# songlab-cal/CherryML

Hardware: AMD Instinct MI355X
Metric: cherry-pairs/sec (whole node) per EM iter (higher is better)
Workload: dtype f64

## Files before the change

cherryml_amd/bank.py:

```python
from typing import Optional, Tuple

import numpy as np

from . import _lib
from ._lib import CB_NO_SYNC, CB_NORMALIZE, CB_PTR_DEVICE, CB_TRAIN_RESUME


def _as_f64(a, shape=None) -> np.ndarray:
    a = np.ascontiguousarray(a, dtype=np.float64)
    if shape is not None and tuple(a.shape) != tuple(shape):
        raise ValueError(f"expected shape {tuple(shape)}, got {a.shape}")
    return a


class CherryBank:

    def __init__(self, t, C, device: int = 0, dtype: str = "f64", per_bucket_products: bool = False):
        self._h = None
        codes = {"f64": _lib.CB_F64, "f32": _lib.CB_F32, "mixed": _lib.CB_MIXED}
        if dtype not in codes:
            raise ValueError(f'dtype must be "f64", "f32" or "mixed", got {dtype!r}')
        self.dtype = dtype
        code = codes[dtype]
        cflags = _lib.CB_PER_BUCKET_PRODUCTS if per_bucket_products else 0
# ... 109 lines not shown
        _lib.check(_lib.load().cb_last_timings(self._h, ms.ctypes.data, ms.size), "cb_last_timings")
        return dict(zip(self.TIMING_NAMES, ms.tolist()))

    def timing_means(self) -> dict:
        import ctypes as Ct
        ms = np.zeros(len(self.TIMING_NAMES))
        calls = Ct.c_int(0)
        _lib.check(_lib.load().cb_timing_sums(self._h, ms.ctypes.data, ms.size, Ct.byref(calls)),
                   "cb_timing_sums")
        k = max(calls.value, 1)
        out = dict(zip(self.TIMING_NAMES, (ms / k).tolist()))
        out["calls"] = calls.value
        return out

    def last_sweeps(self) -> int:
        return int(_lib.load().cb_last_sweeps(self._h))

    def eigh_counters(self) -> dict:
        v = np.zeros(4, dtype=np.int32)
        _lib.check(_lib.load().cb_eigh_counters(self._h, v.ctypes.data, 4), "cb_eigh_counters")
        return {"planned_solves": int(v[0]), "stalls": int(v[1]), "last_sweeps": int(v[2]), "record_spins": int(v[3])}

    def epoch_times(self, num_epochs: int) -> np.ndarray:
        s = np.zeros(int(num_epochs))
        _lib.check(_lib.load().cb_train_epoch_times(self._h, s.ctypes.data, s.size), "cb_train_epoch_times")
        return s

    def last_kernel_form(self) -> int:
        return int(_lib.load().cb_last_kernel_form(self._h))

    def last_bank_form(self) -> dict:
        v = int(_lib.load().cb_last_bank_form(self._h))
        return {"fused": bool(v & 1), "waves_per_tile": 8 if v & 2 else 4, "bucket_sum_first": bool(v & 4),
                "time_basis": bool(v & 8)}

    def time_basis_info(self) -> dict:
        import ctypes as Ct
        n = np.zeros(5, dtype=np.int32)
        rho = Ct.c_double(0.0)
        _lib.check(_lib.load().cb_time_basis_info(self._h, n.ctypes.data, Ct.byref(rho)), "cb_time_basis_info")
        return {"forward_skeleton": int(n[0]), "direct": int(n[1]), "gradient_skeleton": int(n[2]), "builds": int(n[3]),
                "repeated_epochs": int(n[4]), "rho_max": float(rho.value)}

    def _shape_Q(self, Q, pi):
        Q = _as_f64(Q).reshape(self.L, self.S, self.S)
        pi = _as_f64(pi).reshape(self.L, self.S)
        return Q, pi

    def loss_grad(self, Q, pi, normalize: bool = True, want_grad: bool = True
                  ) -> Tuple[np.ndarray, Optional[np.ndarray]]:
        Q, pi = self._shape_Q(Q, pi)
        loss = np.zeros(self.L)
        dQ = np.zeros_like(Q) if want_grad else None
        rc = _lib.load().cb_loss_grad(self._h, Q.ctypes.data, pi.ctypes.data,
                                      CB_NORMALIZE if normalize else 0, loss.ctypes.data,
                                      dQ.ctypes.data if want_grad else None)
        _lib.check(rc, "cb_loss_grad")
        return loss, dQ

    def expm_bank(self, Q, pi=None) -> np.ndarray:
        Q = _as_f64(Q).reshape(self.L, self.S, self.S)
        pi_ptr = None
        if pi is not None:
            pi = _as_f64(pi).reshape(self.L, self.S)
            pi_ptr = pi.ctypes.data
        P = np.zeros((self.L, self.B, self.S, self.S))
        _lib.check(_lib.load().cb_expm_bank(self._h, Q.ctypes.data, pi_ptr, 0, P.ctypes.data),
# ... 84 lines not shown
```

cherryml_amd/csrc/cb_internal.hip.h:

```cpp
#pragma once
#include "../../include/cherrybank.h"

#include <hip/hip_runtime.h>

#include <algorithm>
#include <atomic>
#include <chrono>
#include <cmath>
#include <cstdarg>
#include <cstdio>
#include <cstdlib>
#include <cstring>
#include <string>
#include <vector>

int cb_fail(int code, const char *fmt, ...);
#define fail cb_fail

#define HIP_TRY(expr)                                                                   \
  do {                                                                                  \
    hipError_t e_ = (expr);                                                             \
    if (e_ != hipSuccess)                                                               \
      return fail(e_ == hipErrorOutOfMemory ? CB_ENOMEM : CB_EHIP, "%s failed: %s (%s:%d)", \
                  #expr, hipGetErrorString(e_), __FILE__, __LINE__);                    \
// ... 5 lines not shown
struct CbSpectral {
  int S = 0, LD = 0;
  const double *A = nullptr, *U = nullptr, *lam = nullptr, *dsq = nullptr, *sigma = nullptr;
};
int cb_internal_spectral(cb_handle h, CbSpectral *out);

int cb_launch_bank_fused(int variant, int kg, const void *args, int grid, hipStream_t stream, hipEvent_t stop);

#define CB_TB_RS_MAX 24
#define CB_TB_RG_MAX 40
struct CbTimeBasisHost {
  int B = 0, ns = 0, nd = 0, ng = 0;
  double rho_max = 0.0;
  double res_s = 0.0, res_g = 0.0;
  std::vector<int> kind;
  std::vector<int> skel_s, direct, skel_g;
  std::vector<double> tf, tg;
  std::vector<double> Ls, Lg;
};
bool cb_tb_build(int B, const double *t, double rho_max, CbTimeBasisHost &out);
struct CbTbEwArgs {
  int S, LD, B, ns, nd, ng;
  int nsmall;
  const double *Ct;
  const double *Psi;
  const double *A;
  const double *t;
  const double *Ls, *Lg;
  double *Gh;
  float *Gh32;
  double *loss_part;
  double inv_n;
  const unsigned long long *skip;
};
int cb_tb_launch_tables(int LD, int ns, int nd, int ng, const double *tf, const double *tg, const double *lam, double *F, double *E,
                        double *H, const unsigned long long *skip, hipStream_t stream);
#define CB_TB_LDS_MAX (144u << 10)
size_t cb_tb_ew_lds_bytes(int B, int ns, int ng);
bool cb_tb_supported(int B, int LD, int ns, int ng);
int cb_tb_prepare_ew(int B, int ns, int ng, size_t *cache);
int cb_tb_launch_ew(const CbTbEwArgs &a, hipStream_t stream, hipEvent_t stop, int *nparts);

static inline const char *cb_test_hook(const char *name) {
  const char *on = getenv("CB_TEST_HOOKS");
  return (on && on[0] == '1') ? getenv(name) : nullptr;
}

struct CbDevBufs {
  std::vector<void *> ptrs;
  ~CbDevBufs() {
    for (void *p : ptrs)
      if (p) (void)hipFree(p);
  }
  template <typename T>
  T *up(const T *host, size_t count, int &rc) {
    void *q = nullptr;
    if (rc != CB_OK) return nullptr;
    if (hipMalloc(&q, (count ? count : 1) * sizeof(T)) != hipSuccess) {
      rc = fail(CB_ENOMEM, "device allocation failed");
      return nullptr;
    }
    ptrs.push_back(q);
    if (host && count && hipMemcpyAsync(q, host, count * sizeof(T), hipMemcpyHostToDevice, 0) != hipSuccess)
      rc = fail(CB_EHIP, "upload failed");
    return static_cast<T *>(q);
  }
};
```

cherryml_amd/csrc/cherrybank.hip:

```cpp
#include "cb_internal.hip.h"

#include "common.hip.h"
#include "jacobi_block.hip.h"
#include "jacobi_wave.hip.h"
#include "large_bank.hip.h"
#include "small_bank.hip.h"
#include "train_small.hip.h"
#include "train_large.hip.h"
#include "general_small.hip.h"
#include "general_large.hip.h"
#include "eigh_planned.hip.h"

#define CB_ABI_VERSION 2

static thread_local std::string g_err;

int cb_fail(int code, const char *fmt, ...) {
  char buf[512];
  va_list ap;
  va_start(ap, fmt);
  vsnprintf(buf, sizeof buf, fmt, ap);
  va_end(ap);
  g_err = buf;
  return code;
// ... 181 lines not shown
      h->tb_next_pending = false;
      int rc = tb_install(h, B, std::move(nb), -1.0);
      if (rc != CB_OK || h->tb_failed) return rc;
      took = true;
    }
    if ((stale && !took) || !tb_in_range(h, B, two_sigma)) return tb_rebuild(h, B, two_sigma);
    return CB_OK;
  }
  double warn = 1.6;
  int lead = CB_TB_LEAD;
  if (const char *w = cb_test_hook("CB_TB_TEST_WARN")) sscanf(w, "%lf %d", &warn, &lead);
  if (h->tb_next_pending && epoch >= h->tb_next_epoch) {
    CbTimeBasisHost nb = h->tb_next.get();
    h->tb_next_pending = false;
    int rc = tb_install(h, B, std::move(nb), -1.0);
    if (rc != CB_OK || h->tb_failed) return rc;
  }
  if (!h->tb_next_pending && !tb_in_range(h, B, two_sigma, warn)) {
    std::vector<double> t(h->t_live_host.begin(), h->t_live_host.begin() + B);
    const double rho = two_sigma * tb_growth();
    h->tb_next = std::async(std::launch::async, [t, rho, B]() {
      CbTimeBasisHost nb;
      if (!cb_tb_build(B, t.data(), rho, nb)) nb = CbTimeBasisHost{};
      return nb;
    });
    h->tb_next_pending = true;
    h->tb_next_epoch = epoch + lead;
  }
  return CB_OK;
}

struct LargeBankForm {
  bool tb = false;
  bool fused = false;
  bool accum = false;
  int kg = 1;
  int n_parts = 1;
  int tiles_k3 = 0;
  int test_no_claim = 0;
  double phi_delta = 0;
};

static LargeBankForm choose_large_form(const cb_bank *h, int B, bool Pd, bool want_grad, bool planned_now) {
  static const int streams = getenv("CB_BANK_STREAMS") ? std::min(4, std::max(1, atoi(getenv("CB_BANK_STREAMS")))) : 1;
  const char *tb_hook = cb_test_hook("CB_BANK_TB"), *fused_hook = cb_test_hook("CB_BANK_FUSED"),
             *unfused_hook = cb_test_hook("CB_BANK_UNFUSED"), *k3_hook = cb_test_hook("CB_BANK_K3"),
             *kg_hook = cb_test_hook("CB_BANK_KG"), *no_claim_hook = cb_test_hook("CB_BANK_TEST_NO_CLAIM"),
             *phi_z_hook = cb_test_hook("CB_PHI_Z");
  const int LD = h->LD, tm = (LD + LG_TM - 1) / LG_TM, tn = (LD + LG_TN - 1) / LG_TN;
  const bool f32 = h->dtype == CB_F32 && !Pd;
  LargeBankForm f;
  const bool form_hooks = fused_hook || unfused_hook || k3_hook || kg_hook || no_claim_hook;
  f.tb = h->sym_counts && !h->per_bucket_products && !h->tb_block && !h->tb_failed && !Pd && want_grad && h->tb_Ls[0] &&
         streams == 1 && (h->dtype == CB_F64 || h->dtype == CB_MIXED) &&
         (tb_hook ? atoi(tb_hook) != 0 : (!form_hooks && B >= CB_TB_MIN_B));
  if (f.tb && planned_now && h->tb.B != B) f.tb = false;
  {
    const size_t nb16 = (size_t)LD / 16, cap = (size_t)B * tm * tn;
    if (nb16 * (nb16 + 1) > cap) f.tb = false;
  }
  f.fused = !Pd && want_grad && !unfused_hook && streams == 1 && h->bank_queue && (fused_hook || B >= CB_BANK_FUSED_MIN_B);
  f.accum = h->sym_counts && !h->per_bucket_products && !Pd && want_grad && h->Yk && streams == 1 && h->dtype == CB_F64 &&
            (k3_hook ? atoi(k3_hook) == 0 : (B >= CB_BANK_SUM_FIRST_MIN_B && h->phi_delta >= 4e-3));
  f.tiles_k3 = f.accum ? 0 : h->sym_counts ? tn * (tn + 1) / 2 : tm * tn;
  f.phi_delta = h->phi_delta;
  if (phi_z_hook) f.phi_delta *= atof(phi_z_hook) / 0.1;
  f.kg = (B < CB_BANK_KG2_MAX_B && !f32) ? 2 : 1;
  if (kg_hook) f.kg = atoi(kg_hook) == 1 ? 1 : 2;
  if (Pd) f.kg = 1;
  if (streams > 1 && h->dtype == CB_F64 && !Pd && want_grad && B >= 4 * streams && !h->comm && !h->profile) f.n_parts = streams;
  f.test_no_claim = no_claim_hook ? 1 : 0;
  return f;
}

struct LargeCall {
  int B;
  const double *t;
  double inv_n;
  double *loss, *dQ, *Pd;
  bool dA_padded, planned_now;
  const unsigned long long *skipw;
  size_t LL;
  int tiles, tiles_k1;
};

template <typename T1, typename TG>
struct BankBufs {
  const T1 *Ut, *A, *F, *Ct;
  TG *Gt, *T;
  const TG *U;
  int variant;
};
template <typename T1, typename TG>
// ... 39 lines not shown
  const int LD = h->LD;
  const LossArgs la{h->loss_part, nparts, h->S, h->dsq, h->dirsum, c.inv_n, c.loss, c.skipw};
  const dim3 red_grid((unsigned)((c.LL + 255) / 256) + 1);
  if (f.accum) {
    hipLaunchKernelGGL(ky_reduce_loss<TG>, red_grid, dim3(256), 0, h->stream, src, YArgs{LD, c.B, c.t, h->E, h->Yk}, la);
    K4Args gl{h->S, LD, h->Yk, h->U, h->Lk, nullptr, nullptr, nullptr};
    gl.skip = c.skipw;
    gl.ystride = c.LL;
    launch_sg(h, gl, 0, 0.0, 0.0, nullptr, nullptr, 1 + CB_PHI_TERMS);
    LAUNCH_STOP(k3_stop, kphi_combine<CB_PHI_TERMS>, dim3((unsigned)((c.LL + 255) / 256)), dim3(256), 0, h->stream, LD, h->Lk,
                h->lam, f.phi_delta, h->Mt, c.skipw);
  } else {
    hipLaunchKernelGGL(k3_reduce_loss<TG>, red_grid, dim3(256), 0, h->stream, src, nb, c.LL, h->Mt, sym_ld, la);
  }
  enqueue_k4(h, c, c.skipw, stop_event(h, EV_K4));
  HIP_TRY(hipGetLastError());
  return CB_OK;
}

template <typename TG>
static int enqueue_tb_bank(cb_bank *h, const LargeBankForm &f, const LargeCall &c) {
  constexpr bool mixed = std::is_same_v<TG, float>;
  const CbTimeBasisHost &bas = h->tb;
  const int S = h->S, LD = h->LD, set = h->tb_set, nf = bas.ns + bas.nd, ng = bas.ng;
  const auto bb = bank_bufs<double, TG>(h);
  if (!c.planned_now && cb_tb_launch_tables(LD, bas.ns, bas.nd, ng, h->tb_tf[set], h->tb_tg[set], h->lam, h->F, h->E, h->H,
                                            c.skipw, h->stream) != 0)
    return fail(CB_EHIP, "tb_tables: launch failed");
  double *psi_buf = mixed ? reinterpret_cast<double *>(h->T32) : h->T;
  K1Args<double> k1{S, LD, nf, h->Vc, h->A, h->tb_tf[set], h->F, h->sigma, h->Ct, psi_buf, h->loss_part, c.inv_n, h->dsq, nullptr, c.skipw};
  LAUNCH_STOP(stop_event(h, EV_K1), (k1_pt_loss_gt<double, double, false, 1, true>), dim3(c.tiles_k1 * nf), dim3(LG4_THREADS), 0,
              h->stream, k1);
  const CbTbEwArgs ew{S, LD, c.B, bas.ns, bas.nd, ng, c.B - bas.nd, h->Ct, psi_buf, h->A, c.t, h->tb_Ls[set], h->tb_Lg[set], h->Gt,
                      mixed ? h->Gt32 : nullptr, h->loss_part, c.inv_n, c.skipw};
  int ew_parts = 0;
  if (cb_tb_launch_ew(ew, h->stream, stop_event(h, EV_K2), &ew_parts) != 0) return fail(CB_EHIP, "tb_ew: launch failed");
  if (mixed) launch_cast_f32(h, c, 0);
  const K2Args<TG> k2{LD, bb.Gt, bb.U, bb.T, c.skipw};
  const K3Args<TG> k3{LD, ng, bb.T, bb.U, h->tb_tg[set], h->lam, h->E, h->H, bb.Gt, 1, c.skipw};
  hipLaunchKernelGGL((k2_t_eq_g_u<TG, 1>), dim3(c.tiles * ng), dim3(LG4_THREADS), 0, h->stream, k2);
  LAUNCH_STOP(stop_event(h, EV_K3), (k3_w_phi<TG, 1>), dim3(c.tiles_k1 * ng), dim3(LG4_THREADS), 0, h->stream, k3);
  return enqueue_tail<TG>(h, f, c, bb.Gt, ng, ew_parts, LD, nullptr);
}

template <typename T1, typename TG>
static int enqueue_fused_bank(cb_bank *h, const LargeBankForm &f, const LargeCall &c) {
  const int S = h->S, LD = h->LD, B = c.B;
  const auto bb = bank_bufs<T1, TG>(h);
  const int total = B * (c.tiles_k1 + c.tiles + f.tiles_k3), grid = std::min(h->bank_slots / f.kg, total);
  const int sym = h->sym_counts ? 1 : 0;
  if (h->profile && h->profile_now) h->ev_rec[EV_K1] = h->ev_rec[EV_K2] = false;
  const hipEvent_t bank_stop = stop_event(h, EV_K3);
  static_assert(sizeof(K123Args<float, float>) == sizeof(K123Args<double, double>) &&
                sizeof(K123Args<double, float>) == sizeof(K123Args<double, double>), "one argument block for all");
  const K123Args<T1, TG> a{{S, LD, B, bb.Ut, bb.A, c.t, bb.F, h->sigma, bb.Ct, bb.Gt, h->loss_part, c.inv_n, h->dsq, nullptr, c.skipw},
                           {LD, bb.Gt, bb.U, bb.T, c.skipw},
                           {LD, B, bb.T, bb.U, c.t, h->lam, h->E, h->H, bb.Gt, sym, c.skipw},
                           {h->bank_queue, B, c.tiles_k1, c.tiles, f.tiles_k3, h->bank_claims, f.test_no_claim}};
  auto *dst = reinterpret_cast<K123Args<T1, TG> *>(h->bank_args);
  hipLaunchKernelGGL((lg_tables<K123Args<T1, TG>>), dim3((unsigned)(((size_t)B * LD + 255) / 256)), dim3(256), 0, h->stream, LD, B,
                     c.t, h->lam, h->sigma, h->F, h->E, h->H, a, dst, grid);
  if (std::is_same_v<TG, float>) launch_cast_f32(h, c, (size_t)B * LD);
  if (cb_launch_bank_fused(bb.variant, f.kg, dst, grid, h->stream, bank_stop) != 0) return fail(CB_EHIP, "k123_bank: launch failed");
  return enqueue_tail<TG>(h, f, c, f.accum ? bb.T : bb.Gt, B, B * c.tiles_k1, h->sym_counts ? LD : 0, nullptr);
}

template <typename T1, typename TG>
static int enqueue_split_bank(cb_bank *h, const LargeBankForm &f, const LargeCall &c) {
  const int S = h->S, LD = h->LD, B = c.B;
  const auto bb = bank_bufs<T1, TG>(h);
  launch_tables(h, c);
  if (std::is_same_v<TG, float>) launch_cast_f32(h, c, (size_t)B * LD);
  const K1Args<T1, TG> k1{S, LD, B, bb.Ut, bb.A, c.t, bb.F, h->sigma, bb.Ct, bb.Gt, h->loss_part, c.inv_n, h->dsq, c.Pd, c.skipw};
// ... 62 lines not shown
  HIP_TRY(hipGetLastError());
  return CB_OK;
}

static int large_eval(cb_bank *h, bool normalize, double *lossd, double *out, bool dA_padded, double *Pd,
                      bool reuse_eigh = false, const EighPlan *plan = nullptr, int plan_first_slot = 0) {
  const int LD = h->LD, B = Pd ? h->B : h->Bl;
  const bool planned_now = plan && h->have_prev;
  LargeBankForm f = choose_large_form(h, B, Pd != nullptr, out != nullptr, planned_now);
  const unsigned long long *skipw = planned_now ? h->ectl + (f.tb ? EC_SKIP : EC_STALL) : nullptr;
  int rc = CB_OK;
  if (planned_now) {
    TbTableArgs tbt;
    if (f.tb) tbt = TbTableArgs{h->tb.ns, h->tb.nd, h->tb.ng, h->tb_tf[h->tb_set], h->tb_tg[h->tb_set], h->F, h->E, h->H};
    rc = enqueue_planned_solve(h, *plan, ++h->eseq, plan_first_slot, f.tb ? h->tb.rho_max : 0.0, tbt);
  }
  else if (!(reuse_eigh && h->have_prev)) rc = large_eigh(h, true);
  if (rc != CB_OK) return rc;
  if (f.tb && !planned_now) {
    double sg = 0.0;
    HIP_TRY(hipMemcpyAsync(&sg, h->sigma, sizeof sg, hipMemcpyDeviceToHost, h->stream));
    HIP_TRY(hipStreamSynchronize(h->stream));
    if (!tb_in_range(h, B, 2.0 * sg)) {
      rc = tb_rebuild(h, B, 2.0 * sg);
      if (rc != CB_OK) return rc;
      if (h->tb_failed) f.tb = false;
    }
  }
  if (f.tb) {
    f.fused = f.accum = false;
    f.kg = 1;
  }
  h->bank_tb = f.tb;
  h->bank_fused = f.fused;
  h->bank_accum = f.accum;
  h->bank_kg = f.kg;
  SlowScope scope_bank("large_eval: tables, bank, K4 enqueue");
  if (!planned_now) mark(h, EV_EIGH);
  const int tm = (LD + LG_TM - 1) / LG_TM, tn = (LD + LG_TN - 1) / LG_TN;
  const LargeCall c{B, Pd ? h->t : h->t_live, normalize ? 1.0 / (h->comm ? h->n_global[0] : h->n_host[0]) : 1.0, lossd, out, Pd,
                    dA_padded, planned_now, skipw, (size_t)LD * LD, tm * tn, tn * (tn + 1) / 2};
  if (f.tb) return h->dtype == CB_MIXED ? enqueue_tb_bank<float>(h, f, c) : enqueue_tb_bank<double>(h, f, c);
  if (f.n_parts > 1) return enqueue_stream_split_bank(h, f, c);
  return with_format(h, Pd != nullptr, [&](auto t1, auto tg) {
    using T1 = decltype(t1);
    using TG = decltype(tg);
    return f.fused ? enqueue_fused_bank<T1, TG>(h, f, c) : enqueue_split_bank<T1, TG>(h, f, c);
  });
}

static int large_loss_grad(cb_bank *h, const double *Qd, const double *pid, bool normalize,
                           double *lossd, double *dQd, double *Pd, bool reuse_eigh = false) {
  const size_t LL = (size_t)h->LD * h->LD;
  if (!(reuse_eigh && h->have_prev))
    hipLaunchKernelGGL(lg_build_A, dim3((unsigned)((LL + 255) / 256)), dim3(256), 0, h->stream, h->S, h->LD,
                       Qd, pid, h->A, h->dsq);
  return large_eval(h, normalize, lossd, dQd, false, Pd, reuse_eigh);
}

static int general_run(cb_bank *h, const double *Qd, int flags, double *lossd, double *dQd,
                       double *Pd);
static int finish_call(cb_bank *h, int flags) {
  if ((flags & CB_PTR_DEVICE) && (flags & CB_NO_SYNC)) return CB_OK;
  HIP_TRY(hipStreamSynchronize(h->stream));
  return CB_OK;
}
// ... 221 lines not shown
  h->profile_every = enable > 1 ? enable : 1;
  h->profile_now = h->profile;
  for (double &x : h->t_sum) x = 0.0;
  h->t_calls = 0;
  h->t_pending = false;
  h->t_pending2 = false;
  return CB_OK;
}

extern "C" int cb_timing_sums(cb_handle h, double *ms_sum, int n, int *calls) {
  if (!h || !ms_sum || !calls) return fail(CB_EINVAL, "cb_timing_sums: NULL argument");
  fold_pending(h);
  for (int i = 0; i < n; ++i) ms_sum[i] = i < CB_T_COUNT ? h->t_sum[i] : 0.0;
  *calls = h->t_calls;
  return CB_OK;
}

extern "C" int cb_last_sweeps(cb_handle h) { return h ? h->last_sweeps : 0; }
#ifdef CB_CLOCK_STAMP
extern "C" int cb_debug_clock_stamps(unsigned long long *out) {
  return hipMemcpyFromSymbol(out, HIP_SYMBOL(cb_clock_stamps), sizeof(unsigned long long) * 3 * 4096 * 6) == hipSuccess ? 0 : -1;
}
#endif

extern "C" int cb_eigh_counters(cb_handle h, int *counts, int n) {
  if (!h || !counts || n < 0) return fail(CB_EINVAL, "cb_eigh_counters: NULL argument");
  const int v[4] = {h->planned_solves, h->planned_stalls, h->last_sweeps,
                    (int)std::min<long long>(h->record_spins, 0x7fffffff)};
  for (int i = 0; i < n && i < 4; ++i) counts[i] = v[i];
  return CB_OK;
}
extern "C" int cb_last_kernel_form(cb_handle h) { return h ? h->last_form : 0; }
extern "C" int cb_last_bank_form(cb_handle h) {
  return h ? (h->bank_fused ? 1 : 0) | (h->bank_kg == 2 ? 2 : 0) | (h->bank_accum ? 4 : 0) | (h->bank_tb ? 8 : 0) : 0;
}
extern "C" int cb_time_basis_info(cb_handle h, int *n, double *rho_max) {
  if (!h || !n || !rho_max) return fail(CB_EINVAL, "cb_time_basis_info: NULL argument");
  n[0] = h->tb.ns;
  n[1] = h->tb.nd;
  n[2] = h->tb.ng;
  n[3] = h->tb_builds;
  n[4] = h->tb_stale_epochs;
  *rho_max = h->tb.rho_max;
  return CB_OK;
}

extern "C" int cb_last_timings(cb_handle h, double *ms, int n) {
  if (!h || !ms) return fail(CB_EINVAL, "cb_last_timings: NULL argument");
  for (int i = 0; i < n; ++i) ms[i] = 0.0;
  double v[CB_T_COUNT];
  int rc = read_phase_times(h, v);
  if (rc != CB_OK) return rc;
  for (int i = 0; i < n && i < CB_T_COUNT; ++i) ms[i] = v[i];
  return CB_OK;
}

static int read_phase_times(cb_bank *h, double (&v)[CB_T_COUNT]) {
  for (double &x : v) x = 0.0;
  if (!h->ev_rec[EV_START]) return fail(CB_EINVAL, "cb_last_timings: no profiled call recorded");
  {
    int last = EV_START;
    for (int i = 0; i <= CB_T_COUNT; ++i)
      if (h->ev_rec[i] && i != EV_END && i != EV_AR) last = i;
    if (h->ev_rec[EV_AR]) last = EV_AR;
    HIP_TRY(hipEventSynchronize(h->ev[last]));
  }
  auto span = [&](int a, int b) -> double {
// ... 24 lines not shown
```

cherryml_amd/csrc/handle_host.hip.h:

```cpp
#pragma once
#include <hip/hip_ext.h>
#include <future>
struct EighSlot {
  int cap = 12;
  int nsq = 0;
  int band_after = 0;
  int so = 0;
  int expect_run = 1, expect_order = 12, expect_sq = 2;
};
struct EighPlan {
  int lead_band = 1;
  int nslots = 0;
  EighSlot slot[EC_MAXREC];
};
struct cb_bank {
  int dev = 0, S = 0, L = 0, B = 0;
  int B_cap = 0;
  hipStream_t xstream[3] = {};
  hipEvent_t ev_fork = nullptr, ev_join[3] = {};
  int tr_epochs = 0;
  uint64_t tr_sig = 0;
  int last_form = 0;
  double tr_pow_b1 = 1.0, tr_pow_b2 = 1.0;
  int dtype = CB_F64;
// ... 36 lines not shown
  unsigned long long poll_seq = 0;
  unsigned long long *ectl = nullptr, *epin = nullptr;
  double *epart = nullptr;
  bool begin_folded = false;
  double *sigma_home = nullptr;
  double *sigma2 = nullptr;
  unsigned long long eseq = 0;
  bool planned_unavailable = false;
  int planned_solves = 0, planned_stalls = 0;
  long long record_spins = 0;
  std::vector<double> epoch_seconds;
  EighPlan eplan;
  int k3_chunk = 0, k3_nchunks = 0;
  double *Yk = nullptr, *Lk = nullptr;
  double phi_delta = 0.0;
  unsigned int *bank_queue = nullptr;
  unsigned char *bank_args = nullptr;
  int bank_slots = 0;
  int bank_claims = 0;
  bool bank_fused = false;
  int bank_kg = 1;
  bool bank_accum = false;
  CbTimeBasisHost tb;
  int tb_set = 0;
  double *tb_Ls[2] = {}, *tb_Lg[2] = {}, *tb_tf[2] = {}, *tb_tg[2] = {};
  std::future<CbTimeBasisHost> tb_next;
  bool tb_next_pending = false;
  int tb_next_epoch = 0;
  size_t tb_ew_lds[4] = {0, 0, 0, 0};
  int tb_builds = 0, tb_stale_epochs = 0;
  bool tb_failed = false;
  bool tb_block = false;
  bool bank_tb = false;
  int last_sweeps = 0;
  double *gn_scratch = nullptr, *gn_partial = nullptr;
  int gn_nw = 0;
  struct {
    double *Qn = nullptr, *QT = nullptr, *colsum = nullptr, *alpha = nullptr, *R = nullptr, *RT = nullptr, *E = nullptr,
           *ET = nullptr, *G = nullptr, *GT = nullptr, *Xbar = nullptr, *lpart = nullptr;
    int *nsq = nullptr;
    int cap_slots = 0;
  } gl;
  std::vector<double> t_host, t_live_host;
  bool have_prev = false;
  double *ws_ptr[16] = {};
  size_t ws_cap[16] = {};
  char *pin = nullptr;
  size_t pin_cap = 0, pin_off = 0;
  bool profile = false;
  int profile_every = 1;
  bool profile_now = false;
  hipEvent_t ev[CB_T_COUNT + 1] = {};
  bool ev_rec[CB_T_COUNT + 1] = {};
  double t_sum[CB_T_COUNT] = {};
  int t_calls = 0;
  bool t_pending = false;
  hipEvent_t ev2[CB_T_COUNT + 1] = {};
  bool ev_rec2[CB_T_COUNT + 1] = {};
  bool t_pending2 = false;
};

static void swap_event_sets(cb_bank *h) {
  for (int i = 0; i <= CB_T_COUNT; ++i) {
    std::swap(h->ev[i], h->ev2[i]);
    std::swap(h->ev_rec[i], h->ev_rec2[i]);
  }
// ... 97 lines not shown
```

cherryml_amd/csrc/large_bank.hip.h:

```cpp
#pragma once
#include "common.hip.h"
#include <type_traits>

#define LG_TM 80
#define LG_TN 80
#define LG_KT 16
#define LG4_THREADS 256

typedef float f4 __attribute__((ext_vector_type(4)));
template <typename T> struct Mfma;
template <> struct Mfma<double> {
  typedef d4 acc_t;
  typedef double2 vec_t;
  static constexpr int VEC = 2;
  static __device__ __forceinline__ acc_t mma(double a, double b, acc_t c) { return mfma_f64(a, b, c); }
  static __device__ __forceinline__ int row(int hi, int r) { return hi + 4 * r; }
  static constexpr int RSTEP = 4;
};
template <> struct Mfma<float> {
  typedef f4 acc_t;
  typedef float4 vec_t;
  static constexpr int VEC = 4;
  static __device__ __forceinline__ acc_t mma(float a, float b, acc_t c) {
    return __builtin_amdgcn_mfma_f32_16x16x4f32(a, b, c, 0, 0, 0);
// ... 28 lines not shown
__device__ __forceinline__ PanelSrc<T> lg4_panel_src(const T *P, int ld, int cols_total, int c0, int tid) {
  constexpr int VEC = Panel<T>::VEC, NL = Panel<T>::NL;
  const int kr = tid >> 4, cq = tid & 15;
  PanelSrc<T> s;
  s.rsrc = __builtin_amdgcn_make_buffer_rsrc(const_cast<T *>(P), 0, 0x7fffffff, 0x00027000);
#pragma unroll
  for (int u = 0; u < NL; ++u) s.voff[u] = (kr * ld + min(c0 + VEC * (cq + 16 * u), cols_total - VEC)) * (int)sizeof(T);
  return s;
}
template <typename T, bool SCALE>
__device__ __forceinline__ void lg4_load_panel(const PanelSrc<T> &src, int ld, int k0, typename Mfma<T>::vec_t (&reg)[Panel<T>::NL],
                                               const T *__restrict__ kscale, T &sc, int tid) {
  typedef typename Mfma<T>::vec_t vec_t;
  constexpr int NL = Panel<T>::NL;
  const int soff = k0 * ld * (int)sizeof(T);
#pragma unroll
  for (int u = 0; u < NL; ++u)
    reg[u] = __builtin_bit_cast(vec_t, __builtin_amdgcn_raw_buffer_load_b128(src.rsrc, src.voff[u], soff, 0));
  if (SCALE) sc = kscale[k0 + (tid >> 4)];
}
template <typename T, bool SCALE>
__device__ __forceinline__ void lg4_store_panel(T *s, const typename Mfma<T>::vec_t (&reg)[Panel<T>::NL], T sc, int tid) {
  typedef typename Mfma<T>::vec_t vec_t;
  constexpr int VEC = Panel<T>::VEC, NL = Panel<T>::NL, LAST = Panel<T>::LAST;
  const int kr = tid >> 4, cq = tid & 15;
  T *row = s + kr * LG_TM + VEC * cq;
#pragma unroll
  for (int u = 0; u < NL; ++u) {
    vec_t v = reg[u];
    if (SCALE) vec_scale(v, sc);
    if (u < NL - 1 || cq < LAST) *reinterpret_cast<vec_t *>(row + 16 * VEC * u) = v;
  }
}
struct BankHooks {
  unsigned int *deferred = nullptr;
  unsigned int *draw = nullptr;
  int *drawn_lds = nullptr;
};

template <int KG> __device__ __forceinline__ bool lg_owns_acc(int kg, int j) { return KG == 1 || (kg == 0) == (j < 3); }
template <int KG> __device__ __forceinline__ bool lg_owns_ax0(int kg) { return KG == 1 || kg == 1; }
template <int KG> __device__ __forceinline__ bool lg_owns_ax1(int kg) { return KG == 1 || kg == 0; }

template <typename T, bool SCALE, bool ZERO = true, int KG = 1>
__device__ __forceinline__ void lg4_gemm_tile(const GemmOperands<T> &g, int m0, int n0, T *sA, T *sB,
                                              typename Mfma<T>::acc_t (&acc)[5], typename Mfma<T>::acc_t &ax0,
                                              typename Mfma<T>::acc_t &ax1, int tid = threadIdx.x,
                                              const BankHooks &hooks = BankHooks{}) {
  static_assert(KG == 1 || KG == 2, "one or two K-groups of four waves");
  static_assert(KG == 1 || ZERO, "the accumulate-onto form exists for four waves only");
  typedef typename Mfma<T>::acc_t acc_t;
  typedef typename Mfma<T>::vec_t vec_t;
  const int wv = __builtin_amdgcn_readfirstlane(tid >> 6);
  const int kg = KG == 1 ? 0 : wv >> 2, wave = wv & 3, t4 = tid & 255;
  const int lane = tid & 63, lo = lane & 15, hi = lane >> 4;
  T *const sAll = sA;
  if (KG > 1) {
    sA += kg * (4 * LG_KT * LG_TM);
    sB += kg * (4 * LG_KT * LG_TM);
  }
  if (ZERO) {
#pragma unroll
    for (int j = 0; j < 5; ++j) acc[j] = acc_t{};
    ax0 = acc_t{};
    ax1 = acc_t{};
  }
  vec_t ra[Panel<T>::NL], rb[Panel<T>::NL];
  T sc = T(1), one = T(1);
  const int nk = g.K / LG_KT, nit = (nk + KG - 1) / KG;
  const PanelSrc<T> srcA = lg4_panel_src<T>(g.A, g.lda, g.M, m0, t4), srcB = lg4_panel_src<T>(g.B, g.ldb, g.N, n0, t4);
  if (kg < nk) {
    lg4_load_panel<T, SCALE>(srcA, g.lda, kg * LG_KT, ra, g.kscale, sc, t4);
    lg4_load_panel<T, false>(srcB, g.ldb, kg * LG_KT, rb, nullptr, one, t4);
  }
  __syncthreads();
  if (kg < nk) {
    lg4_store_panel<T, SCALE>(sA, ra, sc, t4);
    lg4_store_panel<T, false>(sB, rb, one, t4);
  }
  unsigned int *deferred = hooks.deferred;
  if (deferred) __builtin_amdgcn_s_waitcnt(0x0F70);
  __syncthreads();
  if (deferred && tid == 0) __hip_atomic_fetch_add(deferred, 1u, __ATOMIC_RELAXED, __HIP_MEMORY_SCOPE_AGENT);
  int drawn = -1;
  const int draw_it = nit > 2 ? 2 / KG : 0;
  for (int it = 0; it < nit; ++it) {
    const int kt = it * KG + kg;
    const T *cA = sA + (it & 1) * (LG_KT * LG_TM), *cB = sB + (it & 1) * (LG_KT * LG_TN);
    if (hooks.draw && it == draw_it && tid == 0)
      drawn = (int)__hip_atomic_fetch_add(hooks.draw, 1u, __ATOMIC_RELAXED, __HIP_MEMORY_SCOPE_AGENT);
    const bool more = kt + KG < nk;
    if (more) {
      lg4_load_panel<T, SCALE>(srcA, g.lda, (kt + KG) * LG_KT, ra, g.kscale, sc, t4);
      lg4_load_panel<T, false>(srcB, g.ldb, (kt + KG) * LG_KT, rb, nullptr, one, t4);
    }
    if (KG == 1 || kt < nk) {
#pragma unroll
      for (int s = 0; s < LG_KT / 4; ++s) {
        const T av = cA[(4 * s + hi) * LG_TM + 16 * wave + lo];
        const T a4 = cA[(4 * s + hi) * LG_TM + 64 + lo];
        T bv[5];
#pragma unroll
        for (int j = 0; j < 5; ++j) bv[j] = cB[(4 * s + hi) * LG_TN + 16 * j + lo];
#pragma unroll
        for (int j = 0; j < 5; ++j) acc[j] = Mfma<T>::mma(av, bv[j], acc[j]);
        const T bx = cB[(4 * s + hi) * LG_TN + 16 * wave + lo];
        ax0 = Mfma<T>::mma(a4, bx, ax0);
        if ((it & 3) == wave) ax1 = Mfma<T>::mma(a4, bv[4], ax1);
      }
    }
    if (more) {
      lg4_store_panel<T, SCALE>(sA + ((it + 1) & 1) * (LG_KT * LG_TM), ra, sc, t4);
      lg4_store_panel<T, false>(sB + ((it + 1) & 1) * (LG_KT * LG_TN), rb, one, t4);
    }
    __syncthreads();
  }
  if (KG == 1) {
    if (wave != 0) {
#pragma unroll
      for (int r = 0; r < 4; ++r) sA[(wave - 1) * 256 + r * 64 + lane] = ax1[r];
    }
    __syncthreads();
    if (wave == 0) {
#pragma unroll
      for (int r = 0; r < 4; ++r) ax1[r] += (sA[r * 64 + lane] + sA[256 + r * 64 + lane]) + sA[512 + r * 64 + lane];
    } else {
      ax1 = acc_t{};
    }
  } else {
    T *px = sAll, *to1 = sAll + 7 * 256, *to0 = to1 + 12 * 256;
    if (wv != 0) {
#pragma unroll
      for (int r = 0; r < 4; ++r) px[(wv - 1) * 256 + r * 64 + lane] = ax1[r];
    }
    if (kg == 0) {
#pragma unroll
      for (int r = 0; r < 4; ++r) {
        to1[(wave * 3 + 0) * 256 + r * 64 + lane] = acc[3][r];
        to1[(wave * 3 + 1) * 256 + r * 64 + lane] = acc[4][r];
        to1[(wave * 3 + 2) * 256 + r * 64 + lane] = ax0[r];
      }
    } else {
#pragma unroll
      for (int r = 0; r < 4; ++r) {
        to0[(wave * 3 + 0) * 256 + r * 64 + lane] = acc[0][r];
        to0[(wave * 3 + 1) * 256 + r * 64 + lane] = acc[1][r];
        to0[(wave * 3 + 2) * 256 + r * 64 + lane] = acc[2][r];
      }
// ... 229 lines not shown
  if (EXPM || RAW) return;
  __syncthreads();
  lossacc = wave_sum(lossacc);
  double *sRed = reinterpret_cast<double *>(sAB);
  if (lane == 0) sRed[wv] = lossacc;
  __syncthreads();
  if (tid == 0) {
    double l = (sRed[0] + sRed[1]) + (sRed[2] + sRed[3]);
    if (KG == 2) l += (sRed[4] + sRed[5]) + (sRed[6] + sRed[7]);
    a.loss_part[vid] = l;
  }
  CB_STAMP_FINISH(0);
}

template <typename T, typename TG = T, bool EXPM = false, int KG = 1, bool RAW = false>
__global__ __launch_bounds__(LG4_THREADS * KG, 4) void k1_pt_loss_gt(K1Args<T, TG> a) {
  if (a.skip && *a.skip != 0ull) return;
  __shared__ T sAB[KG * 4 * LG_KT * LG_TM];
  const int tilesN = (a.LD + LG_TN - 1) / LG_TN, tiles = tilesN * (tilesN + 1) / 2;
  const int vid = xcd_swizzle(blockIdx.x, gridDim.x);
  const int b = vid / tiles;
  k1_tile<T, TG, EXPM, false, KG, RAW>(a, b, vid - b * tiles, sAB, threadIdx.x);
}

template <typename T>
struct K2Args {
  int LD;
  const T *Gt;
  const T *U;
  T *Tm;
  const unsigned long long *skip = nullptr;
};

template <typename T, bool WT, int KG = 1>
__device__ __forceinline__ void k2_tile(const K2Args<T> &a, int b, int tile, T *sAB, int tid, const BankHooks &hooks = BankHooks{}) {
  T *sA = sAB, *sB = sAB + 2 * LG_KT * LG_TM;
  typedef typename Mfma<T>::acc_t acc_t;
  const int tilesN = (a.LD + LG_TN - 1) / LG_TN;
  const int tm = tile / tilesN, tn = tile - tm * tilesN;
  const int m0 = tm * LG_TM, n0 = tn * LG_TN;
  const size_t boff = (size_t)b * a.LD * a.LD;
  GemmOperands<T> g{a.Gt + boff, a.U, a.LD, a.LD, a.LD, a.LD, a.LD, nullptr};
  acc_t acc[5], ax0, ax1;
  CB_STAMP_BEGIN(b * tilesN * tilesN + tile);
  lg4_gemm_tile<T, false, true, KG>(g, m0, n0, sA, sB, acc, ax0, ax1, tid, hooks);
  CB_STAMP_END(1);
  T *__restrict__ Tm = a.Tm + boff;
  lg_for_each<T, KG>(m0, n0, acc, ax0, ax1, [&](int row, int col, T v) {
    if (row < a.LD && col < a.LD) bank_store<WT>(&Tm[(size_t)row * a.LD + col], v);
  }, tid);
  CB_STAMP_FINISH(1);
}

template <typename T, int KG = 1>
__global__ __launch_bounds__(LG4_THREADS * KG, 4) void k2_t_eq_g_u(K2Args<T> a) {
  if (a.skip && *a.skip != 0ull) return;
  __shared__ T sAB[KG * 4 * LG_KT * LG_TM];
  const int tilesN = (a.LD + LG_TN - 1) / LG_TN, tiles = tilesN * tilesN;
  const int vid = xcd_swizzle(blockIdx.x, gridDim.x);
  const int b = vid / tiles;
  k2_tile<T, false, KG>(a, b, vid - b * tiles, sAB, threadIdx.x);
}

template <typename T>
struct K3Args {
  int LD, B;
  const T *Tm;
  const T *U;
  const double *t;
  const double *lam;
  const double *E;
  const double *H;
  T *W;
  int sym;
  const unsigned long long *skip = nullptr;
};

template <typename T, int KG = 1>
__device__ __forceinline__ void k3_tile(const K3Args<T> &a, int b, int tile, T *sAB, int tid, const BankHooks &hooks = BankHooks{}) {
  T *sA = sAB, *sB = sAB + 2 * LG_KT * LG_TM;
  typedef typename Mfma<T>::acc_t acc_t;
  const int tilesN = (a.LD + LG_TN - 1) / LG_TN;
  int tm, tn;
  if (a.sym) {
    tm = 0;
    while (tile >= tilesN - tm) {
      tile -= tilesN - tm;
      ++tm;
    }
    tn = tm + tile;
  } else {
    tm = tile / tilesN;
    tn = tile - tm * tilesN;
  }
// ... 584 lines not shown
```

cherryml_amd/csrc/tbasis.hip.h:

```cpp
#pragma once
#include "cb_internal.hip.h"
#include "common.hip.h"
#include <hip/hip_ext.h>

namespace tbasis {

typedef long double ld;

static inline ld g_phi2(ld x) {
  if (fabsl(x) < 0.5L) {
    ld p = 1.0L;
    for (int k = 24; k >= 3; --k) p = 1.0L + p * x / (ld)k;
    return 0.5L * p;
  }
  return (expm1l(x) - x) / (x * x);
}

static inline ld dot4(const ld *a, const ld *b, int n) {
  ld s0 = 0.0L, s1 = 0.0L, s2 = 0.0L, s3 = 0.0L;
  int i = 0;
  for (; i + 3 < n; i += 4) {
    s0 += a[i] * b[i];
    s1 += a[i + 1] * b[i + 1];
    s2 += a[i + 2] * b[i + 2];
// ... 320 lines not shown
      const bool in = b >= nsm && b < B;
      const double v = __builtin_bit_cast(double, __builtin_amdgcn_raw_buffer_load_b64(rp, (int)((unsigned)(in ? b - nsm : 0) * plane) + eoff, 0, 0));
      pp[m] = in ? v : 1.0;
    }
  };
  double c0[4] = {0.0, 0.0, 0.0, 0.0}, c1[4] = {0.0, 0.0, 0.0, 0.0}, p0[4] = {1.0, 1.0, 1.0, 1.0}, p1[4] = {1.0, 1.0, 1.0, 1.0};
  load(0, c0, p0);
  for (int b0 = 0; b0 < B; b0 += 32) {
    load(b0 + 16, c1, p1);
    tb_ew_step<RS, RG>(b0, j, k, nsm, sLs, sLg, sT, ltab, psi, a_e, dl, a.inv_n, c0, p0, D, loss, bad);
    if (b0 + 16 >= B) break;
    load(b0 + 32, c0, p0);
    tb_ew_step<RS, RG>(b0 + 16, j, k, nsm, sLs, sLg, sT, ltab, psi, a_e, dl, a.inv_n, c1, p1, D, loss, bad);
  }
  if (live) {
    if (a.Gh32) {
      float *__restrict__ Gh = a.Gh32 + e;
#pragma unroll
      for (int q = 0; q < RG / 16; ++q)
#pragma unroll
        for (int r = 0; r < 4; ++r) {
          const int rr = 16 * q + k + 4 * r;
          if (rr < a.ng) Gh[(size_t)rr * LL] = (float)D[q][r];
        }
    } else {
      double *__restrict__ Gh = a.Gh + e;
#pragma unroll
      for (int q = 0; q < RG / 16; ++q)
#pragma unroll
        for (int r = 0; r < 4; ++r) {
          const int rr = 16 * q + k + 4 * r;
          if (rr < a.ng) Gh[(size_t)rr * LL] = D[q][r];
        }
    }
  } else {
    loss = 0.0;
    bad = 0;
  }
  if (bad) loss = NAN;
  loss = wave_sum(loss) * lossw;
  if (lane == 0) sred[wave] = loss;
  __syncthreads();
  if (tid == 0) {
    double s = 0.0;
    for (int w = 0; w < NWAVE; ++w) s += sred[w];
    a.loss_part[blockIdx.x] = s;
  }
}

template <typename T>
__global__ __launch_bounds__(256) void tb_mirror(int LD, T *__restrict__ Gh, const unsigned long long *skip) {
  __shared__ T tile[16][17];
  if (skip && *skip != 0ull) return;
  const int nb = LD / 16;
  int I = 0, rest = (int)blockIdx.x;
  while (rest >= nb - 1 - I) {
    rest -= nb - 1 - I;
    ++I;
  }
  const int J = I + 1 + rest, r = threadIdx.x >> 4, c = threadIdx.x & 15;
  T *G = Gh + (size_t)blockIdx.y * LD * LD;
  tile[r][c] = G[(size_t)(16 * I + r) * LD + 16 * J + c];
  __syncthreads();
  G[(size_t)(16 * J + r) * LD + 16 * I + c] = tile[c][r];
}

// ... 13 lines not shown
  const int RS = ns <= 16 ? 16 : 24, RG = ng <= 32 ? 32 : 48;
  const int BP = (B + 15) & ~15;
  return ((size_t)BP * (RS + 1 + RG + 2 + 1) + 256 + 16) * sizeof(double);
}

int cb_tb_prepare_ew(int B, int ns, int ng, size_t *cache) {
#define TB_PREP(RS_, RG_, slot_)                                                                                         \
  do {                                                                                                                   \
    const size_t lds = (size_t)TbEwLds<RS_, RG_>(B).TOTAL * sizeof(double);                                              \
    if (lds > cache[slot_]) {                                                                                            \
      if (hipFuncSetAttribute(reinterpret_cast<const void *>(tb_ew<RS_, RG_, 8, true>), hipFuncAttributeMaxDynamicSharedMemorySize, (int)lds) != hipSuccess) { \
        (void)hipGetLastError();                                                                                         \
        return -1;                                                                                                       \
      }                                                                                                                  \
      cache[slot_] = lds;                                                                                                \
    }                                                                                                                    \
  } while (0)
  if (ns <= 16 && ng <= 32) TB_PREP(16, 32, 0);
  else if (ns <= 16) TB_PREP(16, 48, 1);
  else if (ng <= 32) TB_PREP(24, 32, 2);
  else TB_PREP(24, 48, 3);
#undef TB_PREP
  return 0;
}

int cb_tb_launch_ew(const CbTbEwArgs &a, hipStream_t stream, hipEvent_t stop, int *nparts) {
  if (!cb_tb_supported(a.B, a.LD, a.ns, a.ng)) return -1;
  const int nb = a.LD / 16, nblk = nb * (nb + 1) / 2;
  const unsigned grid = (unsigned)(nblk * 2);
  if (nparts) *nparts = (int)grid;
#define TB_GO(RS_, RG_)                                                                                                  \
  do {                                                                                                                   \
    const size_t lds = (size_t)TbEwLds<RS_, RG_>(a.B).TOTAL * sizeof(double);                                            \
    hipLaunchKernelGGL((tb_ew<RS_, RG_, 8, true>), dim3(grid), dim3(512), lds, stream, a);                               \
  } while (0)
  if (a.ns <= 16 && a.ng <= 32) TB_GO(16, 32);
  else if (a.ns <= 16) TB_GO(16, 48);
  else if (a.ng <= 32) TB_GO(24, 32);
  else TB_GO(24, 48);
#undef TB_GO
  if (nb > 1) {
    const dim3 mg((unsigned)(nb * (nb - 1) / 2), (unsigned)a.ng);
    if (a.Gh32) {
      if (stop) hipExtLaunchKernelGGL(tb_mirror<float>, mg, dim3(256), 0, stream, nullptr, stop, 0, a.LD, a.Gh32, a.skip);
      else hipLaunchKernelGGL(tb_mirror<float>, mg, dim3(256), 0, stream, a.LD, a.Gh32, a.skip);
    } else {
      if (stop) hipExtLaunchKernelGGL(tb_mirror<double>, mg, dim3(256), 0, stream, nullptr, stop, 0, a.LD, a.Gh, a.skip);
      else hipLaunchKernelGGL(tb_mirror<double>, mg, dim3(256), 0, stream, a.LD, a.Gh, a.skip);
    }
  } else if (stop) {
    (void)hipEventRecord(stop, stream);
  }
  return hipGetLastError() == hipSuccess ? 0 : -1;
}
```

Measured before the change: 1.550 billion.

## Drop tb_mirror pass by exploiting symmetric G in K2 and in-tile mirror stores

In the f64 time-basis path, the tb_mirror kernel that copied the upper triangle of Gh into the lower triangle is removed. tb_ew now writes mirrored 16x16 blocks only when they fall inside the same K2 row tile. K2 instead reads the A panels that lie beyond the diagonal tile in transposed form from the upper triangle, relying on G being symmetric. This saves one kernel launch and a full pass of mirror writes, at the cost of strided transposed panel loads in K2 and extra scattered stores in tb_ew.

```diff
diff --git a/cherryml_amd/bank.py b/cherryml_amd/bank.py
--- a/cherryml_amd/bank.py
+++ b/cherryml_amd/bank.py
@@ -165,7 +165,7 @@
     def last_bank_form(self) -> dict:
         v = int(_lib.load().cb_last_bank_form(self._h))
         return {"fused": bool(v & 1), "waves_per_tile": 8 if v & 2 else 4, "bucket_sum_first": bool(v & 4),
-                "time_basis": bool(v & 8)}
+                "time_basis": bool(v & 8), "mirror_free": bool(v & 16)}
 
     def time_basis_info(self) -> dict:
         import ctypes as Ct
diff --git a/cherryml_amd/csrc/cb_internal.hip.h b/cherryml_amd/csrc/cb_internal.hip.h
--- a/cherryml_amd/csrc/cb_internal.hip.h
+++ b/cherryml_amd/csrc/cb_internal.hip.h
@@ -61,6 +61,7 @@
   double *loss_part;
   double inv_n;
   const unsigned long long *skip;
+  int mirror_tile;
 };
 int cb_tb_launch_tables(int LD, int ns, int nd, int ng, const double *tf, const double *tg, const double *lam, double *F, double *E,
                         double *H, const unsigned long long *skip, hipStream_t stream);
@@ -73,6 +74,10 @@
 static inline const char *cb_test_hook(const char *name) {
   const char *on = getenv("CB_TEST_HOOKS");
   return (on && on[0] == '1') ? getenv(name) : nullptr;
+}
+static inline bool cb_epoch_legacy_launches() {
+  const char *v = cb_test_hook("CB_EPOCH_LEGACY_LAUNCHES");
+  return v && atoi(v) != 0;
 }
 
 struct CbDevBufs {
diff --git a/cherryml_amd/csrc/cherrybank.hip b/cherryml_amd/csrc/cherrybank.hip
--- a/cherryml_amd/csrc/cherrybank.hip
+++ b/cherryml_amd/csrc/cherrybank.hip
@@ -237,6 +237,7 @@
 
 struct LargeBankForm {
   bool tb = false;
+  bool tb_sym_a = false;
   bool fused = false;
   bool accum = false;
   int kg = 1;
@@ -264,6 +265,7 @@
     const size_t nb16 = (size_t)LD / 16, cap = (size_t)B * tm * tn;
     if (nb16 * (nb16 + 1) > cap) f.tb = false;
   }
+  f.tb_sym_a = h->dtype == CB_F64 && LD % LG_TM == 0 && !cb_epoch_legacy_launches();
   f.fused = !Pd && want_grad && !unfused_hook && streams == 1 && h->bank_queue && (fused_hook || B >= CB_BANK_FUSED_MIN_B);
   f.accum = h->sym_counts && !h->per_bucket_products && !Pd && want_grad && h->Yk && streams == 1 && h->dtype == CB_F64 &&
             (k3_hook ? atoi(k3_hook) == 0 : (B >= CB_BANK_SUM_FIRST_MIN_B && h->phi_delta >= 4e-3));
@@ -369,13 +371,18 @@
   LAUNCH_STOP(stop_event(h, EV_K1), (k1_pt_loss_gt<double, double, false, 1, true>), dim3(c.tiles_k1 * nf), dim3(LG4_THREADS), 0,
               h->stream, k1);
   const CbTbEwArgs ew{S, LD, c.B, bas.ns, bas.nd, ng, c.B - bas.nd, h->Ct, psi_buf, h->A, c.t, h->tb_Ls[set], h->tb_Lg[set], h->Gt,
-                      mixed ? h->Gt32 : nullptr, h->loss_part, c.inv_n, c.skipw};
+                      mixed ? h->Gt32 : nullptr, h->loss_part, c.inv_n, c.skipw, (!mixed && f.tb_sym_a) ? LG_TM / 16 : 0};
   int ew_parts = 0;
   if (cb_tb_launch_ew(ew, h->stream, stop_event(h, EV_K2), &ew_parts) != 0) return fail(CB_EHIP, "tb_ew: launch failed");
   if (mixed) launch_cast_f32(h, c, 0);
   const K2Args<TG> k2{LD, bb.Gt, bb.U, bb.T, c.skipw};
   const K3Args<TG> k3{LD, ng, bb.T, bb.U, h->tb_tg[set], h->lam, h->E, h->H, bb.Gt, 1, c.skipw};
-  hipLaunchKernelGGL((k2_t_eq_g_u<TG, 1>), dim3(c.tiles * ng), dim3(LG4_THREADS), 0, h->stream, k2);
+  if constexpr (!mixed) {
+    if (f.tb_sym_a) hipLaunchKernelGGL((k2_t_eq_g_u<double, 1, true>), dim3(c.tiles * ng), dim3(LG4_THREADS), 0, h->stream, k2);
+    else hipLaunchKernelGGL((k2_t_eq_g_u<double, 1>), dim3(c.tiles * ng), dim3(LG4_THREADS), 0, h->stream, k2);
+  } else {
+    hipLaunchKernelGGL((k2_t_eq_g_u<float, 1>), dim3(c.tiles * ng), dim3(LG4_THREADS), 0, h->stream, k2);
+  }
   LAUNCH_STOP(stop_event(h, EV_K3), (k3_w_phi<TG, 1>), dim3(c.tiles_k1 * ng), dim3(LG4_THREADS), 0, h->stream, k3);
   return enqueue_tail<TG>(h, f, c, bb.Gt, ng, ew_parts, LD, nullptr);
 }
@@ -504,6 +511,7 @@
     f.kg = 1;
   }
   h->bank_tb = f.tb;
+  h->bank_tb_sym_a = f.tb && f.tb_sym_a;
   h->bank_fused = f.fused;
   h->bank_accum = f.accum;
   h->bank_kg = f.kg;
@@ -791,7 +799,9 @@
 }
 extern "C" int cb_last_kernel_form(cb_handle h) { return h ? h->last_form : 0; }
 extern "C" int cb_last_bank_form(cb_handle h) {
-  return h ? (h->bank_fused ? 1 : 0) | (h->bank_kg == 2 ? 2 : 0) | (h->bank_accum ? 4 : 0) | (h->bank_tb ? 8 : 0) : 0;
+  return h ? (h->bank_fused ? 1 : 0) | (h->bank_kg == 2 ? 2 : 0) | (h->bank_accum ? 4 : 0) | (h->bank_tb ? 8 : 0) |
+                 (h->bank_tb_sym_a ? 16 : 0)
+           : 0;
 }
 extern "C" int cb_time_basis_info(cb_handle h, int *n, double *rho_max) {
   if (!h || !n || !rho_max) return fail(CB_EINVAL, "cb_time_basis_info: NULL argument");
diff --git a/cherryml_amd/csrc/handle_host.hip.h b/cherryml_amd/csrc/handle_host.hip.h
--- a/cherryml_amd/csrc/handle_host.hip.h
+++ b/cherryml_amd/csrc/handle_host.hip.h
@@ -92,6 +92,7 @@
   bool tb_failed = false;
   bool tb_block = false;
   bool bank_tb = false;
+  bool bank_tb_sym_a = false;
   int last_sweeps = 0;
   double *gn_scratch = nullptr, *gn_partial = nullptr;
   int gn_nw = 0;
diff --git a/cherryml_amd/csrc/large_bank.hip.h b/cherryml_amd/csrc/large_bank.hip.h
--- a/cherryml_amd/csrc/large_bank.hip.h
+++ b/cherryml_amd/csrc/large_bank.hip.h
@@ -84,6 +84,35 @@
     if (u < NL - 1 || cq < LAST) *reinterpret_cast<vec_t *>(row + 16 * VEC * u) = v;
   }
 }
+struct PanelSrcTr {
+  int voff[3];
+  int lds;
+};
+__device__ __forceinline__ PanelSrcTr lg4_panel_src_tr(int ld, int m0, int tid) {
+  const int ml = tid & 15, c = (tid >> 4) & 7, mh = tid >> 7;
+  PanelSrcTr s;
+#pragma unroll
+  for (int u = 0; u < 3; ++u) s.voff[u] = ((m0 + ml + 16 * min(mh + 2 * u, 4)) * ld + 2 * c) * (int)sizeof(double);
+  s.lds = 2 * c * LG_TM + ml + 16 * mh;
+  return s;
+}
+template <typename T>
+__device__ __forceinline__ void lg4_load_panel_tr(__amdgpu_buffer_rsrc_t rsrc, const PanelSrcTr &src, int k0,
+                                                  typename Mfma<T>::vec_t (&reg)[Panel<T>::NL]) {
+  typedef typename Mfma<T>::vec_t vec_t;
+  const int soff = k0 * (int)sizeof(T);
+#pragma unroll
+  for (int u = 0; u < Panel<T>::NL; ++u) reg[u] = __builtin_bit_cast(vec_t, __builtin_amdgcn_raw_buffer_load_b128(rsrc, src.voff[u], soff, 0));
+}
+template <typename T>
+__device__ __forceinline__ void lg4_store_panel_tr(T *s, const PanelSrcTr &src, const typename Mfma<T>::vec_t (&reg)[Panel<T>::NL], int tid) {
+#pragma unroll
+  for (int u = 0; u < Panel<T>::NL; ++u)
+    if (u < 2 || tid < 128) {
+      s[src.lds + 32 * u] = reg[u].x;
+      s[src.lds + 32 * u + LG_TM] = reg[u].y;
+    }
+}
 struct BankHooks {
   unsigned int *deferred = nullptr;
   unsigned int *draw = nullptr;
@@ -94,13 +123,14 @@
 template <int KG> __device__ __forceinline__ bool lg_owns_ax0(int kg) { return KG == 1 || kg == 1; }
 template <int KG> __device__ __forceinline__ bool lg_owns_ax1(int kg) { return KG == 1 || kg == 0; }
 
-template <typename T, bool SCALE, bool ZERO = true, int KG = 1>
+template <typename T, bool SCALE, bool ZERO = true, int KG = 1, bool SYMA = false>
 __device__ __forceinline__ void lg4_gemm_tile(const GemmOperands<T> &g, int m0, int n0, T *sA, T *sB,
                                               typename Mfma<T>::acc_t (&acc)[5], typename Mfma<T>::acc_t &ax0,
                                               typename Mfma<T>::acc_t &ax1, int tid = threadIdx.x,
                                               const BankHooks &hooks = BankHooks{}) {
   static_assert(KG == 1 || KG == 2, "one or two K-groups of four waves");
   static_assert(KG == 1 || ZERO, "the accumulate-onto form exists for four waves only");
+  static_assert(!SYMA || (std::is_same_v<T, double> && KG == 1 && !SCALE && ZERO), "the symmetric A operand: float64, four waves, no row scale");
   typedef typename Mfma<T>::acc_t acc_t;
   typedef typename Mfma<T>::vec_t vec_t;
   const int wv = __builtin_amdgcn_readfirstlane(tid >> 6);
@@ -121,6 +151,8 @@
   T sc = T(1), one = T(1);
   const int nk = g.K / LG_KT, nit = (nk + KG - 1) / KG;
   const PanelSrc<T> srcA = lg4_panel_src<T>(g.A, g.lda, g.M, m0, t4), srcB = lg4_panel_src<T>(g.B, g.ldb, g.N, n0, t4);
+  [[maybe_unused]] PanelSrcTr srcT{};
+  if constexpr (SYMA) srcT = lg4_panel_src_tr(g.lda, m0, t4);
   if (kg < nk) {
     lg4_load_panel<T, SCALE>(srcA, g.lda, kg * LG_KT, ra, g.kscale, sc, t4);
     lg4_load_panel<T, false>(srcB, g.ldb, kg * LG_KT, rb, nullptr, one, t4);
@@ -136,17 +168,48 @@
   if (deferred && tid == 0) __hip_atomic_fetch_add(deferred, 1u, __ATOMIC_RELAXED, __HIP_MEMORY_SCOPE_AGENT);
   int drawn = -1;
   const int draw_it = nit > 2 ? 2 / KG : 0;
-  for (int it = 0; it < nit; ++it) {
-    const int kt = it * KG + kg;
-    const T *cA = sA + (it & 1) * (LG_KT * LG_TM), *cB = sB + (it & 1) * (LG_KT * LG_TN);
-    if (hooks.draw && it == draw_it && tid == 0)
-      drawn = (int)__hip_atomic_fetch_add(hooks.draw, 1u, __ATOMIC_RELAXED, __HIP_MEMORY_SCOPE_AGENT);
-    const bool more = kt + KG < nk;
-    if (more) {
-      lg4_load_panel<T, SCALE>(srcA, g.lda, (kt + KG) * LG_KT, ra, g.kscale, sc, t4);
-      lg4_load_panel<T, false>(srcB, g.ldb, (kt + KG) * LG_KT, rb, nullptr, one, t4);
-    }
-    if (KG == 1 || kt < nk) {
+  if constexpr (!SYMA) {
+    for (int it = 0; it < nit; ++it) {
+      const int kt = it * KG + kg;
+      const T *cA = sA + (it & 1) * (LG_KT * LG_TM), *cB = sB + (it & 1) * (LG_KT * LG_TN);
+      if (hooks.draw && it == draw_it && tid == 0)
+        drawn = (int)__hip_atomic_fetch_add(hooks.draw, 1u, __ATOMIC_RELAXED, __HIP_MEMORY_SCOPE_AGENT);
+      const bool more = kt + KG < nk;
+      if (more) {
+        lg4_load_panel<T, SCALE>(srcA, g.lda, (kt + KG) * LG_KT, ra, g.kscale, sc, t4);
+        lg4_load_panel<T, false>(srcB, g.ldb, (kt + KG) * LG_KT, rb, nullptr, one, t4);
+      }
+      if (KG == 1 || kt < nk) {
+#pragma unroll
+        for (int s = 0; s < LG_KT / 4; ++s) {
+          const T av = cA[(4 * s + hi) * LG_TM + 16 * wave + lo];
+          const T a4 = cA[(4 * s + hi) * LG_TM + 64 + lo];
+          T bv[5];
+#pragma unroll
+          for (int j = 0; j < 5; ++j) bv[j] = cB[(4 * s + hi) * LG_TN + 16 * j + lo];
+#pragma unroll
+          for (int j = 0; j < 5; ++j) acc[j] = Mfma<T>::mma(av, bv[j], acc[j]);
+          const T bx = cB[(4 * s + hi) * LG_TN + 16 * wave + lo];
+          ax0 = Mfma<T>::mma(a4, bx, ax0);
+          if ((it & 3) == wave) ax1 = Mfma<T>::mma(a4, bv[4], ax1);
+        }
+      }
+      if (more) {
+        lg4_store_panel<T, SCALE>(sA + ((it + 1) & 1) * (LG_KT * LG_TM), ra, sc, t4);
+        lg4_store_panel<T, false>(sB + ((it + 1) & 1) * (LG_KT * LG_TN), rb, one, t4);
+      }
+      __syncthreads();
+    }
+  } else {
+    auto k_step = [&](int it, auto tr_next) {
+      constexpr bool TRN = decltype(tr_next)::value;
+      const T *cA = sA + (it & 1) * (LG_KT * LG_TM), *cB = sB + (it & 1) * (LG_KT * LG_TN);
+      const bool more = it + 1 < nk;
+      if (more) {
+        if constexpr (TRN) lg4_load_panel_tr<T>(srcA.rsrc, srcT, (it + 1) * LG_KT, ra);
+        else lg4_load_panel<T, false>(srcA, g.lda, (it + 1) * LG_KT, ra, nullptr, one, t4);
+        lg4_load_panel<T, false>(srcB, g.ldb, (it + 1) * LG_KT, rb, nullptr, one, t4);
+      }
 #pragma unroll
       for (int s = 0; s < LG_KT / 4; ++s) {
         const T av = cA[(4 * s + hi) * LG_TM + 16 * wave + lo];
@@ -160,12 +223,17 @@
         ax0 = Mfma<T>::mma(a4, bx, ax0);
         if ((it & 3) == wave) ax1 = Mfma<T>::mma(a4, bv[4], ax1);
       }
-    }
-    if (more) {
-      lg4_store_panel<T, SCALE>(sA + ((it + 1) & 1) * (LG_KT * LG_TM), ra, sc, t4);
-      lg4_store_panel<T, false>(sB + ((it + 1) & 1) * (LG_KT * LG_TN), rb, one, t4);
-    }
-    __syncthreads();
+      if (more) {
+        if constexpr (TRN) lg4_store_panel_tr<T>(sA + ((it + 1) & 1) * (LG_KT * LG_TM), srcT, ra, t4);
+        else lg4_store_panel<T, false>(sA + ((it + 1) & 1) * (LG_KT * LG_TM), ra, one, t4);
+        lg4_store_panel<T, false>(sB + ((it + 1) & 1) * (LG_KT * LG_TN), rb, one, t4);
+      }
+      __syncthreads();
+    };
+    const int n_dir = min((m0 + LG_TM) / LG_KT - 1, nk);
+    int it = 0;
+    for (; it < n_dir; ++it) k_step(it, std::false_type{});
+    for (; it < nk; ++it) k_step(it, std::true_type{});
   }
   if (KG == 1) {
     if (wave != 0) {
@@ -461,7 +529,7 @@
   const unsigned long long *skip = nullptr;
 };
 
-template <typename T, bool WT, int KG = 1>
+template <typename T, bool WT, int KG = 1, bool SYMA = false>
 __device__ __forceinline__ void k2_tile(const K2Args<T> &a, int b, int tile, T *sAB, int tid, const BankHooks &hooks = BankHooks{}) {
   T *sA = sAB, *sB = sAB + 2 * LG_KT * LG_TM;
   typedef typename Mfma<T>::acc_t acc_t;
@@ -472,7 +540,7 @@
   GemmOperands<T> g{a.Gt + boff, a.U, a.LD, a.LD, a.LD, a.LD, a.LD, nullptr};
   acc_t acc[5], ax0, ax1;
   CB_STAMP_BEGIN(b * tilesN * tilesN + tile);
-  lg4_gemm_tile<T, false, true, KG>(g, m0, n0, sA, sB, acc, ax0, ax1, tid, hooks);
+  lg4_gemm_tile<T, false, true, KG, SYMA>(g, m0, n0, sA, sB, acc, ax0, ax1, tid, hooks);
   CB_STAMP_END(1);
   T *__restrict__ Tm = a.Tm + boff;
   lg_for_each<T, KG>(m0, n0, acc, ax0, ax1, [&](int row, int col, T v) {
@@ -481,14 +549,14 @@
   CB_STAMP_FINISH(1);
 }
 
-template <typename T, int KG = 1>
+template <typename T, int KG = 1, bool SYMA = false>
 __global__ __launch_bounds__(LG4_THREADS * KG, 4) void k2_t_eq_g_u(K2Args<T> a) {
   if (a.skip && *a.skip != 0ull) return;
   __shared__ T sAB[KG * 4 * LG_KT * LG_TM];
   const int tilesN = (a.LD + LG_TN - 1) / LG_TN, tiles = tilesN * tilesN;
   const int vid = xcd_swizzle(blockIdx.x, gridDim.x);
   const int b = vid / tiles;
-  k2_tile<T, false, KG>(a, b, vid - b * tiles, sAB, threadIdx.x);
+  k2_tile<T, false, KG, SYMA>(a, b, vid - b * tiles, sAB, threadIdx.x);
 }
 
 template <typename T>
diff --git a/cherryml_amd/csrc/tbasis.hip.h b/cherryml_amd/csrc/tbasis.hip.h
--- a/cherryml_amd/csrc/tbasis.hip.h
+++ b/cherryml_amd/csrc/tbasis.hip.h
@@ -376,6 +376,28 @@
           const int rr = 16 * q + k + 4 * r;
           if (rr < a.ng) Gh[(size_t)rr * LL] = D[q][r];
         }
+      if (SYM && a.mirror_tile > 0) {
+        const int nb = a.LD / 16, item = __builtin_amdgcn_readfirstlane((int)blockIdx.x * NWAVE + wave), rr = item & 15;
+        int I = 0, rest = item >> 4;
+        while (rest >= nb - I) {
+          rest -= nb - I;
+          ++I;
+        }
+        const int J = I + rest;
+        if (J > I && I / a.mirror_tile == J / a.mirror_tile) {
+          typedef unsigned int u2 __attribute__((ext_vector_type(2)));
+          const __amdgpu_buffer_rsrc_t rg = __builtin_amdgcn_make_buffer_rsrc(a.Gh, 0, 0x7fffffff, 0x00027000);
+          const int vm = (int)((unsigned)k * plane) + ((16 * J + j) * a.LD + 16 * I + rr) * (int)sizeof(double);
+#pragma unroll
+          for (int q = 0; q < RG / 16; ++q)
+#pragma unroll
+            for (int r = 0; r < 4; ++r)
+              if (16 * q + k + 4 * r < a.ng) {
+                const double v = D[q][r];
+                __builtin_amdgcn_raw_buffer_store_b64(__builtin_bit_cast(u2, v), rg, vm, (int)((unsigned)(16 * q + 4 * r) * plane), 0);
+              }
+        }
+      }
     }
   } else {
     loss = 0.0;
@@ -455,13 +477,16 @@
 #define TB_GO(RS_, RG_)                                                                                                  \
   do {                                                                                                                   \
     const size_t lds = (size_t)TbEwLds<RS_, RG_>(a.B).TOTAL * sizeof(double);                                            \
-    hipLaunchKernelGGL((tb_ew<RS_, RG_, 8, true>), dim3(grid), dim3(512), lds, stream, a);                               \
+    if (stop && a.mirror_tile > 0)                                                                                       \
+      hipExtLaunchKernelGGL((tb_ew<RS_, RG_, 8, true>), dim3(grid), dim3(512), lds, stream, nullptr, stop, 0, a);        \
+    else hipLaunchKernelGGL((tb_ew<RS_, RG_, 8, true>), dim3(grid), dim3(512), lds, stream, a);                          \
   } while (0)
   if (a.ns <= 16 && a.ng <= 32) TB_GO(16, 32);
   else if (a.ns <= 16) TB_GO(16, 48);
   else if (a.ng <= 32) TB_GO(24, 32);
   else TB_GO(24, 48);
 #undef TB_GO
+  if (a.mirror_tile > 0) return hipGetLastError() == hipSuccess ? 0 : -1;
   if (nb > 1) {
     const dim3 mg((unsigned)(nb * (nb - 1) / 2), (unsigned)a.ng);
     if (a.Gh32) {
```

Result: no change. 1.538 billion (-0.8%).
